# sidfeels/cosmos-predict2.5

Measured on AMD Instinct MI355X. Metric: frames/sec, Predict2.5-2B Image2World 720p×121f, 35 UniPC steps, CP=1/8, higher is better.
Workload: dtype bf16

## Files before the change

cosmos-predict2.5_amd/csrc/attn_wide.hip:

```cpp
#include "attn_common.h"

namespace cp25attn {
namespace {

constexpr int kAheadWq = 2;
constexpr int kRingWq = kAheadWq + 1;
static_assert(kWqThreads == 4 * 64, "one wave per SIMD");

constexpr int wq_stage(int nq) { return 17 * nq; }
constexpr int wq_frag(int nq, int m) { return m < nq ? -1 : (m - nq) / nq; }
constexpr int wq_qb(int nq, int m) { return m < nq ? m : (m - nq) % nq; }
constexpr bool wq_read_gap(int nq, int m) { return m >= nq && (m - nq) % nq == 0; }
constexpr int wq_sm_op(int nq, int m) {
  if (wq_read_gap(nq, m)) return -1;
  int idx = 0;
  for (int x = 0; x < m; ++x) idx += !wq_read_gap(nq, x);
  return idx < 12 * nq ? idx : -1;
}
constexpr int wq_sm_count(int nq) {
  int n = 0;
  for (int m = 0; m < wq_stage(nq); ++m) n += wq_sm_op(nq, m) >= 0;
  return n;
}
static_assert(wq_sm_count(5) == 60 && wq_sm_count(6) == 72, "every softmax instruction has a gap");
constexpr int wq_dma_at(int nq, int M) {
  return M < wq_stage(nq) && wq_read_gap(nq, M) && wq_frag(nq, M) < 10 ? wq_frag(nq, M) : -1;
}
constexpr int wq_m0_at(int nq, int M) { return wq_dma_at(nq, M + 1); }

__device__ __forceinline__ u32x4 tile_rsrc(const char* base, int64_t sl, int rows) {
  const uint64_t p = (uint64_t)base;
  const unsigned n = rows > 0 ? (unsigned)((rows - 1) * sl * 2 + 2 * kD) : 0u;
  return u32x4{(unsigned)p, (unsigned)(p >> 32) & 0xffffu, n, 0x00020000u};
}

#define WQ_MFMA "v_mfma_f32_16x16x32_bf16 "

template <int kNQ, int kMode, int kTail = 0>
__global__ void __launch_bounds__(kWqThreads, 1) attn_fwd_wq(AttnArgs a) {
  static_assert(kMode == 0 || kMode == 1, "kMode: 0 fixed shift, 1 zero shift");
  static_assert(kNQ >= 4 && kNQ <= 6, "query blocks per wave");
  __shared__ __attribute__((aligned(16))) char smem[kLds16];
  constexpr bool kInit = kMode != 1;
  constexpr int KB1 = kKBuf16, VB0 = 2 * kKBuf16;
  constexpr int kR = kRingWq;
  constexpr int kRowsW = 16 * kNQ;
  constexpr int kRowsG = 4 * kRowsW;
  constexpr int kNS = wq_stage(kNQ);
  constexpr int kQA = (256 - 36 * kNQ - 4) / 16 < kNQ ? (256 - 36 * kNQ - 4) / 16 : kNQ;

  const int tile = xcd_remap(blockIdx.x, gridDim.x);
  const int qblk = tile % a.nqb;
  const int bhs = tile / a.nqb;
  const int split = bhs % a.nsplit, bh = bhs / a.nsplit;
  const int b = bh / a.H, h = bh % a.H;
  const int key0 = split * a.tps * kKBlk;
  const int Lk = min(a.Lk - key0, a.tps * kKBlk);
  const int ntk = (Lk + kKBlk - 1) / kKBlk;
  const int tid = threadIdx.x;
  const int lane = tid & 63;
  const int wave = __builtin_amdgcn_readfirstlane(tid >> 6);
  const int c16 = lane & 15;
  const int g = lane >> 4;
  const int row_w = qblk * kRowsG + wave * kRowsW;

  const unsigned short* qp = a.q + b * a.q_sb + h * a.q_sh;
  const char* const kbase = (const char*)(a.k + b * a.k_sb + h * a.k_sh + (int64_t)key0 * a.k_sl);
  const char* const vbase = (const char*)(a.v + b * a.v_sb + h * a.v_sh + (int64_t)key0 * a.v_sl);

  int dk[5], dv[5];
#pragma unroll
  for (int j = 0; j < 5; ++j) {
    const int bb = 1024 * (wave + 4 * j) + 16 * lane;
    const int row = bb / kKStride16, cb = bb - row * kKStride16;
    dk[j] = cb < 2 * kD ? row * (int)(a.k_sl * 2) + cb : 0;
    dv[j] = cb < 2 * kD ? row * (int)(a.v_sl * 2) + cb : 0;
  }
  const unsigned lds_wave = (unsigned)(uintptr_t)(lds_char_ptr)smem + 1024u * (unsigned)wave;
  auto k_rsrc = [&](int t) __attribute__((always_inline)) {
    return tile_rsrc(kbase + (int64_t)t * kKBlk * a.k_sl * 2, a.k_sl, min(Lk - t * kKBlk, kKBlk));
  };
  auto v_rsrc = [&](int t) __attribute__((always_inline)) {
    return tile_rsrc(vbase + (int64_t)t * kKBlk * a.v_sl * 2, a.v_sl, min(Lk - t * kKBlk, kKBlk));
  };
  auto set_m0 = [&](unsigned dst, auto OFFC) __attribute__((always_inline)) {
    asm volatile("s_add_u32 m0, %0, %1" ::"s"(dst), "i"(decltype(OFFC)::value) : "memory");
  };
  auto dma_load = [&](const u32x4& rs, int off) __attribute__((always_inline)) {
    asm volatile("buffer_load_dwordx4 %0, %1, 0 offen lds" ::"v"(off), "s"(rs) : "memory");
  };
  auto dma_tile = [&](const u32x4& rs, const int* offs, unsigned dst) __attribute__((always_inline)) {
    static_for<5>([&](auto JC) __attribute__((always_inline)) {
      constexpr int j = decltype(JC)::value;
      if (j < 4 || wave < 2) {
        set_m0(dst, std::integral_constant<int, 4096 * j>{});
        asm volatile("s_nop 0" ::: "memory");
        dma_load(rs, offs[j]);
      }
    });
  };

  dma_tile(k_rsrc(0), dk, lds_wave);
  dma_tile(k_rsrc(1), dk, lds_wave + KB1);
  dma_tile(v_rsrc(0), dv, lds_wave + VB0);

  bf16x8 qa[kNQ][4];
#pragma unroll
  for (int qb = 0; qb < kNQ; ++qb) {
    const int r = row_w + 16 * qb + c16;
    const unsigned short* src = qp + (int64_t)min(r, a.Lq - 1) * a.q_sl + 8 * g;
#pragma unroll
    for (int s = 0; s < 4; ++s) qa[qb][s] = *reinterpret_cast<const bf16x8*>(src + 32 * s);
  }
  if (a.qn_w != nullptr) {
    bf16x8 wv[4];
#pragma unroll
    for (int s = 0; s < 4; ++s) wv[s] = *reinterpret_cast<const bf16x8*>(a.qn_w + 32 * s + 8 * g);
    const bool rope = a.qn_cos != nullptr;
    const f32x2 scale2 = {a.qn_scale, a.qn_scale};
#pragma unroll
    for (int qb = 0; qb < kNQ; ++qb) {
      const int r = row_w + 16 * qb + c16;
      f32x4 rc[2][2], rsn[2][2];
      if (rope) {
        const int64_t t0 = (a.qn_row0 + min(r, a.Lq - 1)) * 64 + 8 * g;
#pragma unroll
        for (int s1 = 0; s1 < 2; ++s1)
#pragma unroll
          for (int hf = 0; hf < 2; ++hf) {
            rc[s1][hf] = *reinterpret_cast<const f32x4*>(a.qn_cos + t0 + 32 * s1 + 4 * hf);
            rsn[s1][hf] = *reinterpret_cast<const f32x4*>(a.qn_sin + t0 + 32 * s1 + 4 * hf);
          }
      }
      f32x2 x[4][4];
#pragma unroll
      for (int s = 0; s < 4; ++s)
#pragma unroll
        for (int q = 0; q < 4; ++q)
          x[s][q] = f32x2{static_cast<float>(qa[qb][s][2 * q]), static_cast<float>(qa[qb][s][2 * q + 1])};
      f32x2 c01[8], c23[8];
#pragma unroll
      for (int e = 0; e < 8; ++e) {
        c01[e] = f32x2{x[0][e >> 1][e & 1], x[1][e >> 1][e & 1]};
        c23[e] = f32x2{x[2][e >> 1][e & 1], x[3][e >> 1][e & 1]};
      }
      const f32x2 p01 = hn2_sumsq8(c01), p23 = hn2_sumsq8(c23);
      const f32x2 aa = p01 + p23;
      float ss = aa.x + aa.y;
      ss += __shfl_xor(ss, 32);
      ss += __shfl_xor(ss, 16);
      const float rstd = hn_rstd(ss, a.qn_eps);
      const f32x2 rstd2 = {rstd, rstd};
#pragma unroll
      for (int s = 0; s < 4; ++s)
#pragma unroll
        for (int q = 0; q < 4; ++q)
          x[s][q] = hn2_norm(x[s][q], rstd2,
                             f32x2{static_cast<float>(wv[s][2 * q]), static_cast<float>(wv[s][2 * q + 1])});
      f32x2 y[4][4];
#pragma unroll
      for (int s = 0; s < 4; ++s)
#pragma unroll
        for (int q = 0; q < 4; ++q) y[s][q] = x[s][q];
      if (rope) {
#pragma unroll
        for (int s = 0; s < 4; ++s)
#pragma unroll
          for (int q = 0; q < 4; ++q) {
            const f32x4 cc = rc[s & 1][q >> 1], sn = rsn[s & 1][q >> 1];
            const int o = 2 * (q & 1);
            y[s][q] = hn2_rope(x[s][q], x[s ^ 2][q], s < 2 ? -1.f : 1.f, f32x2{cc[o], cc[o + 1]},
                               f32x2{sn[o], sn[o + 1]});
          }
      }
#pragma unroll
      for (int s = 0; s < 4; ++s)
#pragma unroll
        for (int q = 0; q < 4; ++q) {
          const bf16x2v hh = __builtin_convertvector(y[s][q] * scale2, bf16x2v);
          qa[qb][s][2 * q] = hh.x;
          qa[qb][s][2 * q + 1] = hh.y;
        }
    }
  }

  float m_run[kNQ];
#pragma unroll
  for (int qb = 0; qb < kNQ; ++qb) m_run[qb] = 0.f;
  if constexpr (kMode == 0) {
#pragma unroll
    for (int qb = 0; qb < kNQ; ++qb) {
      float qq = 0.f;
#pragma unroll
      for (int s = 0; s < 4; ++s)
#pragma unroll
        for (int e = 0; e < 8; ++e) {
          const float x = static_cast<float>(qa[qb][s][e]);
          qq = fmaf(x, x, qq);
        }
      const float b_row = sqrtf(group4_sum(qq)) * a.kbound;
      m_run[qb] = floorf(fminf(b_row + kPDrop, 126.f - b_row));
    }
  }
  f32x4 minit[kNQ];
#pragma unroll
  for (int qb = 0; qb < kNQ; ++qb) {
    minit[qb] = f32x4{-m_run[qb], -m_run[qb], -m_run[qb], -m_run[qb]};
    asm volatile("" : "+v"(minit[qb]));
  }

  f32x4 oacc[8][kNQ], lacc[kNQ];
#pragma unroll
  for (int db = 0; db < 8; ++db)
#pragma unroll
    for (int qb = 0; qb < kNQ; ++qb) {
      oacc[db][qb] = f32x4{0.f, 0.f, 0.f, 0.f};
      asm volatile("s_nop 2" : "+a"(oacc[db][qb]));
    }
#pragma unroll
  for (int qb = 0; qb < kNQ; ++qb) {
    lacc[qb] = f32x4{0.f, 0.f, 0.f, 0.f};
    asm volatile("s_nop 2" : "+a"(lacc[qb]));
  }
  static_for<kNQ>([&](auto QC) __attribute__((always_inline)) {
    constexpr int qb = decltype(QC)::value;
    (void)qa;
#pragma unroll
    for (int s = 0; s < 4; ++s) {
      if constexpr (qb < kQA) asm volatile("s_nop 2" : "+a"(qa[qb][s]));
      else asm volatile("s_nop 2" : "+v"(qa[qb][s]));
    }
  });
  typedef short s16x8v __attribute__((ext_vector_type(8)));
  bf16x8 ones8 = __builtin_bit_cast(bf16x8, s16x8v{0x3f80, 0x3f80, 0x3f80, 0x3f80, 0x3f80, 0x3f80, 0x3f80, 0x3f80});
  asm volatile("s_nop 2" : "+a"(ones8));
  const unsigned k_rd_lds = (unsigned)(uintptr_t)(lds_char_ptr)(smem + c16 * kKStride16 + 16 * g);
  const unsigned v_rd_lds =
      (unsigned)(uintptr_t)(lds_char_ptr)(smem + VB0 + (4 * g + (c16 >> 2)) * kVStride16 + 8 * (c16 & 3));

  f32x4 S[2][2][kNQ];
  bf16x8 P[2][kNQ];
  bf16x8 ring[kR];
  float ex[2];
  unsigned pk[4];
  unsigned k_cur = 0, v_cur = 0;

  auto issue = [&](auto FC, auto SLOTC) __attribute__((always_inline)) {
    constexpr int F = decltype(FC)::value, slot = decltype(SLOTC)::value;
    constexpr int st = F / 16, f = F % 16;
    (void)ring;
    (void)k_cur;
    (void)v_cur;
    if constexpr (f >= 8) {
      constexpr int j = f - 8;
      constexpr int off = (2 * st + (j & 1)) * 16 * kKStride16 + 64 * (j >> 1);
      asm volatile("ds_read_b128 %0, %1 offset:%2" : "=v"(ring[slot]) : "v"(k_cur), "i"(off));
    } else {
      constexpr int off = 32 * st * kVStride16 + 32 * f;
      s16x4 lo, hi;
      asm volatile("ds_read_b64_tr_b16 %0, %1 offset:%2" : "=v"(lo) : "v"(v_cur), "i"(off));
      asm volatile("ds_read_b64_tr_b16 %0, %1 offset:%2" : "=v"(hi) : "v"(v_cur), "i"(off + 16 * kVStride16));
      typedef short s16x8 __attribute__((ext_vector_type(8)));
      const s16x8 r = {lo[0], lo[1], lo[2], lo[3], hi[0], hi[1], hi[2], hi[3]};
      ring[slot] = __builtin_bit_cast(bf16x8, r);
    }
  };

  auto mask_keys = [&](auto SPC, int k0) __attribute__((always_inline)) {
    constexpr int SP = decltype(SPC)::value;
    if (__builtin_expect(k0 + 32 > Lk, 0)) {
      asm volatile("s_nop 15\n\ts_nop 15" ::: "memory");
#pragma unroll
      for (int kbl = 0; kbl < 2; ++kbl)
#pragma unroll
        for (int i = 0; i < 4; ++i)
          if (k0 + 16 * kbl + 4 * g + i >= Lk) {
#pragma unroll
            for (int qb = 0; qb < kNQ; ++qb) S[SP][kbl][qb][i] = -INFINITY;
          }
    }
  };

  auto body = [&](auto FULLC, int t) __attribute__((always_inline)) {
    constexpr bool FULL = decltype(FULLC)::value;
    constexpr int NF = FULL ? 32 : 16;
    constexpr auto frag_of = [](int n) constexpr { return FULL ? n : (n < 8 ? 8 + n : 16 + n); };
    constexpr auto seq_of = [](int F) constexpr { return FULL ? F : (F < 16 ? F - 8 : F - 16); };
    constexpr auto nreads = [](int F) constexpr { return F % 16 < 8 ? 2 : 1; };
    k_cur = k_rd_lds + (((t + 1) & 1) ? (unsigned)KB1 : 0u);
    v_cur = v_rd_lds + ((t & 1) ? (unsigned)kVBuf16 : 0u);
    u32x4 rk = {0u, 0u, 0u, 0u}, rv = {0u, 0u, 0u, 0u};
    unsigned dst_k = 0, dst_v = 0;
    if constexpr (FULL) {
      mask_keys(std::integral_constant<int, 1>{}, 64 * t + 32);
      rk = k_rsrc(t + 2);
      rv = v_rsrc(t + 1);
      dst_k = lds_wave + ((t & 1) ? (unsigned)KB1 : 0u);
      dst_v = lds_wave + (unsigned)VB0 + (((t + 1) & 1) ? (unsigned)kVBuf16 : 0u);
    }
    static_for<kAheadWq>([&](auto IC) __attribute__((always_inline)) {
      constexpr int n = decltype(IC)::value;
      issue(std::integral_constant<int, frag_of(n)>{}, std::integral_constant<int, n % kR>{});
    });
    __builtin_amdgcn_sched_barrier(0);
    static_for<2 * kNS>([&](auto MC) __attribute__((always_inline)) {
      constexpr int M = decltype(MC)::value;
      constexpr int st = M / kNS, m = M % kNS;
      constexpr int f = wq_frag(kNQ, m), qb = wq_qb(kNQ, m);
      constexpr int F = 16 * st + (f < 0 ? 0 : f);
      constexpr bool has_mfma = f >= 8 || FULL;
      constexpr bool has_sm = st == 1 || FULL;
      (void)S;
      (void)ex;
      (void)pk;
      (void)oacc;
      (void)lacc;
      (void)ones8;
      (void)P;
      (void)minit;
      (void)qa;
      (void)ring;
      (void)rk;
      (void)rv;
      (void)dst_k;
      (void)dst_v;
      if constexpr (m == 0 && st == 1) {
        if constexpr (!FULL) asm volatile("s_nop 15" ::: "memory");
        mask_keys(std::integral_constant<int, 0>{}, 64 * (t + 1));
        __builtin_amdgcn_sched_barrier(0);
      }
      if constexpr (has_mfma) {
        if constexpr (f >= 0 && qb == 0) {
          constexpr int n = seq_of(F);
          constexpr int pending = [=]() constexpr {
            int p = 0;
            for (int i = 1; i < kAheadWq; ++i)
              if (n + i < NF) p += nreads(frag_of(n + i));
            return p;
          }();
          asm volatile("s_waitcnt lgkmcnt(%0)" ::"i"(pending), "v"(ring[n % kR]) : "memory");
        }
        if constexpr (f < 0) {
          asm volatile(WQ_MFMA "%0, %1, %2, %0" : "+a"(lacc[qb]) : "a"(ones8), "v"(P[st][qb]));
        } else if constexpr (f < 8) {
          asm volatile(WQ_MFMA "%0, %1, %2, %0" : "+a"(oacc[f][qb]) : "v"(ring[seq_of(F) % kR]), "v"(P[st][qb]));
        } else {
          constexpr int kbl = (f - 8) & 1, s = (f - 8) >> 1;
          constexpr int ri = seq_of(F) % kR;
          if constexpr (qb < kQA) {
            if constexpr (s == 0 && kInit)
              asm volatile(WQ_MFMA "%0, %1, %2, %3"
                           : "=&v"(S[st][kbl][qb]) : "v"(ring[ri]), "a"(qa[qb][s]), "v"(minit[qb]));
            else if constexpr (s == 0)
              asm volatile(WQ_MFMA "%0, %1, %2, 0" : "=&v"(S[st][kbl][qb]) : "v"(ring[ri]), "a"(qa[qb][s]));
            else
              asm volatile(WQ_MFMA "%0, %1, %2, %0" : "+v"(S[st][kbl][qb]) : "v"(ring[ri]), "a"(qa[qb][s]));
          } else {
            if constexpr (s == 0 && kInit)
              asm volatile(WQ_MFMA "%0, %1, %2, %3"
                           : "=&v"(S[st][kbl][qb]) : "v"(ring[ri]), "v"(qa[qb][s]), "v"(minit[qb]));
            else if constexpr (s == 0)
              asm volatile(WQ_MFMA "%0, %1, %2, 0" : "=&v"(S[st][kbl][qb]) : "v"(ring[ri]), "v"(qa[qb][s]));
            else
              asm volatile(WQ_MFMA "%0, %1, %2, %0" : "+v"(S[st][kbl][qb]) : "v"(ring[ri]), "v"(qa[qb][s]));
          }
        }
      }
      __builtin_amdgcn_sched_barrier(0);
      if constexpr (has_mfma && f >= 0 && qb == 0) {
        constexpr int n = seq_of(F) + kAheadWq;
        if constexpr (n < NF) issue(std::integral_constant<int, frag_of(n)>{}, std::integral_constant<int, n % kR>{});
      }
      if constexpr (FULL) {
        constexpr int dm = wq_m0_at(kNQ, M), dl = wq_dma_at(kNQ, M);
        if constexpr (dm >= 0) {
          constexpr int j = dm % 5;
          if (j < 4 || wave < 2) set_m0(dm < 5 ? dst_k : dst_v, std::integral_constant<int, 4096 * j>{});
        }
        if constexpr (dl >= 0) {
          constexpr int j = dl % 5;
          if (j < 4 || wave < 2) dma_load(dl < 5 ? rk : rv, dl < 5 ? dk[j] : dv[j]);
        }
      }
      if constexpr (has_sm) {
        if constexpr (!has_mfma) asm volatile("s_nop 1" ::: "memory");
        constexpr int op = wq_sm_op(kNQ, m);
        if constexpr (op >= 0) {
          constexpr int q = op / 12, r = op % 12, pair = r / 3, w = r % 3;
          if constexpr (w < 2) {
            constexpr int j = 2 * pair + w;
            asm volatile("v_exp_f32 %0, %1" : "=v"(ex[w]) : "v"(S[1 - st][j >> 2][q][j & 3]));
          } else {
            pk[pair] = __builtin_bit_cast(unsigned, __builtin_convertvector(f32x2{ex[0], ex[1]}, bf16x2v));
            asm volatile("" ::"v"(pk[pair]));
            if constexpr (pair == 3) P[1 - st][q] = __builtin_bit_cast(bf16x8, u32x4{pk[0], pk[1], pk[2], pk[3]});
          }
        }
      }
      __builtin_amdgcn_sched_barrier(0);
    });
    if constexpr (FULL) {
      static_for<kNQ>([&](auto QC) __attribute__((always_inline)) {
        constexpr int qb = decltype(QC)::value;
        (void)P;
        asm volatile("" ::"v"(P[0][qb]), "v"(P[1][qb]));
      });
    }
    asm volatile("s_waitcnt vmcnt(0)" ::: "memory");
    __builtin_amdgcn_s_barrier();
    __builtin_amdgcn_sched_barrier(0);
  };

  asm volatile("s_waitcnt vmcnt(0) lgkmcnt(0)" ::: "memory");
  __builtin_amdgcn_s_barrier();
  body(std::false_type{}, -1);
  for (int t = 0; t < ntk; ++t) body(std::true_type{}, t);

  asm volatile("s_nop 15\n\ts_nop 15" ::: "memory");
#pragma unroll
  for (int db = 0; db < 8; ++db)
#pragma unroll
    for (int qb = 0; qb < kNQ; ++qb) asm volatile("s_nop 0" : "+a"(oacc[db][qb]));
#pragma unroll
  for (int qb = 0; qb < kNQ; ++qb) asm volatile("s_nop 0" : "+a"(lacc[qb]));
#pragma unroll
  for (int qb = 0; qb < kNQ; ++qb) {
    const int q_row = row_w + 16 * qb + c16;
    const float l_tot = lacc[qb][0];
    float inv = 1.f / l_tot;
    if (l_tot > 3.0e38f) inv = __uint_as_float(0x7fc00000u);
    if (q_row >= a.Lq) continue;
    if (a.nsplit > 1) {
      const int64_t row = ((int64_t)(split * a.B + b) * a.H + h) * a.Lq + q_row;
      float* op = a.o_part + row * kD + 4 * g;
#pragma unroll
      for (int db = 0; db < 8; ++db) {
        f32x4 w;
#pragma unroll
        for (int e = 0; e < 4; ++e) w[e] = oacc[db][qb][e] * inv;
        *reinterpret_cast<f32x4*>(op + 16 * db) = w;
      }
      if (g == 0) a.lse_part[row] = m_run[qb] + __log2f(l_tot);
    } else {
      unsigned short* op = a.o + b * a.o_sb + h * a.o_sh + (int64_t)q_row * a.o_sl + 4 * g;
#pragma unroll
      for (int db = 0; db < 8; ++db) {
        u16x4 w;
#pragma unroll
        for (int e = 0; e < 4; ++e) w[e] = f2bf(oacc[db][qb][e] * inv);
        *reinterpret_cast<u16x4*>(op + 16 * db) = w;
      }
    }
  }
}

#undef WQ_MFMA

}

AttnKernel wq_kernel(int rows, int mode, bool tail) {
  if (mode != 0) return nullptr;
  if (rows == 320) return tail ? attn_fwd_wq<5, 0, 1> : attn_fwd_wq<5, 0>;
  if (rows == 384) return tail ? attn_fwd_wq<6, 0, 1> : attn_fwd_wq<6, 0>;
  return nullptr;
}

}
```

Before: 0.7987.

## Process two key tiles per barrier iteration in wide-query attention kernel

Restructures the attention main loop so each iteration consumes two K/V tiles instead of one, doubling the LDS staging buffers and halving the number of s_waitcnt/s_barrier synchronisations per key range. The DMA schedule is regenerated for 18 loads per iteration, with the fifth (partial) image piece split across wave pairs. Buffer resource descriptors are computed at the iteration head by default. The goal is less barrier and pipeline-drain overhead, at the cost of more LDS, longer unrolled code and a new tile-count rounding for odd tile counts.

```diff
diff --git a/cosmos-predict2.5_amd/csrc/attn_wide.hip b/cosmos-predict2.5_amd/csrc/attn_wide.hip
--- a/cosmos-predict2.5_amd/csrc/attn_wide.hip
+++ b/cosmos-predict2.5_amd/csrc/attn_wide.hip
@@ -23,10 +23,36 @@
   return n;
 }
 static_assert(wq_sm_count(5) == 60 && wq_sm_count(6) == 72, "every softmax instruction has a gap");
-constexpr int wq_dma_at(int nq, int M) {
-  return M < wq_stage(nq) && wq_read_gap(nq, M) && wq_frag(nq, M) < 10 ? wq_frag(nq, M) : -1;
-}
-constexpr int wq_m0_at(int nq, int M) { return wq_dma_at(nq, M + 1); }
+#ifdef CP25_WQ_PARENT_LOOP
+#define CP25_WQ_ITER_TILES 1
+#undef CP25_WQ_NO_PAD_FETCH
+#undef CP25_WQ_GAP_RSRC
+#endif
+#ifndef CP25_WQ_ITER_TILES
+#define CP25_WQ_ITER_TILES 2
+#endif
+constexpr int wq_iter_tiles(int) { return CP25_WQ_ITER_TILES; }
+#ifdef CP25_WQ_NO_PAD_FETCH
+constexpr bool kWqPadFetch = false;
+#else
+constexpr bool kWqPadFetch = true;
+#endif
+#ifdef CP25_WQ_GAP_RSRC
+constexpr bool kWqHeadRsrc = false;
+#else
+constexpr bool kWqHeadRsrc = true;
+#endif
+constexpr int kWqImg = kKBuf16;
+static_assert(kKBuf16 == kVBuf16, "K and V images of one size");
+constexpr int wq_dma_n(int it) { return it == 1 ? 10 : 18; }
+constexpr int wq_dma_at(int nq, int it, int M) {
+  const int st = M / wq_stage(nq), m = M % wq_stage(nq);
+  if (st >= 2 * it || !wq_read_gap(nq, m)) return -1;
+  const int F = 16 * st + wq_frag(nq, m);
+  return F < wq_dma_n(it) ? F : -1;
+}
+constexpr int wq_m0_at(int nq, int it, int M) { return wq_dma_at(nq, it, M + 1); }
+constexpr int kWqNoFetch = 0x7ffffff0;
 
 __device__ __forceinline__ u32x4 tile_rsrc(const char* base, int64_t sl, int rows) {
   const uint64_t p = (uint64_t)base;
@@ -40,9 +66,15 @@
 __global__ void __launch_bounds__(kWqThreads, 1) attn_fwd_wq(AttnArgs a) {
   static_assert(kMode == 0 || kMode == 1, "kMode: 0 fixed shift, 1 zero shift");
   static_assert(kNQ >= 4 && kNQ <= 6, "query blocks per wave");
-  __shared__ __attribute__((aligned(16))) char smem[kLds16];
+  constexpr int kIT = wq_iter_tiles(kNQ);
+  static_assert(kIT == 1 || kIT == 2, "tiles per iteration");
+  constexpr int kBuf = kIT * kWqImg;
+  constexpr int VB0 = 2 * kBuf;
+  static_assert(4 * kBuf <= 163840, "the CU's LDS");
+  __shared__ __attribute__((aligned(16))) char smem[4 * kBuf];
   constexpr bool kInit = kMode != 1;
-  constexpr int KB1 = kKBuf16, VB0 = 2 * kKBuf16;
+  constexpr int kPar = kIT == 1 ? 1 : 0;
+  constexpr int kND = wq_dma_n(kIT);
   constexpr int kR = kRingWq;
   constexpr int kRowsW = 16 * kNQ;
   constexpr int kRowsG = 4 * kRowsW;
@@ -68,15 +100,19 @@
   const char* const kbase = (const char*)(a.k + b * a.k_sb + h * a.k_sh + (int64_t)key0 * a.k_sl);
   const char* const vbase = (const char*)(a.v + b * a.v_sb + h * a.v_sh + (int64_t)key0 * a.v_sl);
 
+  const int wave5 = kIT == 1 ? wave : (wave & 1);
+  const int img5 = kIT == 1 ? 0 : (wave >> 1);
   int dk[5], dv[5];
 #pragma unroll
   for (int j = 0; j < 5; ++j) {
-    const int bb = 1024 * (wave + 4 * j) + 16 * lane;
+    const int bb = 1024 * ((j < 4 ? wave : wave5) + 4 * j) + 16 * lane;
     const int row = bb / kKStride16, cb = bb - row * kKStride16;
-    dk[j] = cb < 2 * kD ? row * (int)(a.k_sl * 2) + cb : 0;
-    dv[j] = cb < 2 * kD ? row * (int)(a.v_sl * 2) + cb : 0;
+    dk[j] = cb < 2 * kD ? row * (int)(a.k_sl * 2) + cb : (kWqPadFetch ? 0 : kWqNoFetch);
+    dv[j] = cb < 2 * kD ? row * (int)(a.v_sl * 2) + cb : (kWqPadFetch ? 0 : kWqNoFetch);
   }
   const unsigned lds_wave = (unsigned)(uintptr_t)(lds_char_ptr)smem + 1024u * (unsigned)wave;
+  const unsigned lds_wave5 =
+      (unsigned)(uintptr_t)(lds_char_ptr)smem + 1024u * (unsigned)wave5 + (unsigned)kWqImg * (unsigned)img5;
   auto k_rsrc = [&](int t) __attribute__((always_inline)) {
     return tile_rsrc(kbase + (int64_t)t * kKBlk * a.k_sl * 2, a.k_sl, min(Lk - t * kKBlk, kKBlk));
   };
@@ -84,25 +120,43 @@
     return tile_rsrc(vbase + (int64_t)t * kKBlk * a.v_sl * 2, a.v_sl, min(Lk - t * kKBlk, kKBlk));
   };
   auto set_m0 = [&](unsigned dst, auto OFFC) __attribute__((always_inline)) {
-    asm volatile("s_add_u32 m0, %0, %1" ::"s"(dst), "i"(decltype(OFFC)::value) : "memory");
+    asm volatile("s_add_u32 m0, %0, %1" ::"s"(dst), "i"(decltype(OFFC)::value) : "memory", "scc");
   };
   auto dma_load = [&](const u32x4& rs, int off) __attribute__((always_inline)) {
     asm volatile("buffer_load_dwordx4 %0, %1, 0 offen lds" ::"v"(off), "s"(rs) : "memory");
   };
-  auto dma_tile = [&](const u32x4& rs, const int* offs, unsigned dst) __attribute__((always_inline)) {
-    static_for<5>([&](auto JC) __attribute__((always_inline)) {
-      constexpr int j = decltype(JC)::value;
-      if (j < 4 || wave < 2) {
-        set_m0(dst, std::integral_constant<int, 4096 * j>{});
-        asm volatile("s_nop 0" ::: "memory");
-        dma_load(rs, offs[j]);
-      }
+  auto dma_piece = [&](const u32x4& rs, int off, unsigned dst, auto OFFC) __attribute__((always_inline)) {
+    set_m0(dst, OFFC);
+    asm volatile("s_nop 4" ::: "memory");
+    dma_load(rs, off);
+  };
+  auto dma_img = [&](const u32x4& rs, const int* offs, unsigned at) __attribute__((always_inline)) {
+    static_for<4>([&](auto JC) __attribute__((always_inline)) {
+      dma_piece(rs, offs[decltype(JC)::value], lds_wave + at, std::integral_constant<int, 4096 * decltype(JC)::value>{});
     });
   };
-
-  dma_tile(k_rsrc(0), dk, lds_wave);
-  dma_tile(k_rsrc(1), dk, lds_wave + KB1);
-  dma_tile(v_rsrc(0), dv, lds_wave + VB0);
+  auto dma_buf = [&](auto rsrc, const int* offs, int t0, unsigned at) __attribute__((always_inline)) {
+    if constexpr (kIT == 1) {
+      const u32x4 rs = rsrc(t0);
+      dma_img(rs, offs, at);
+      if (wave < 2) dma_piece(rs, offs[4], lds_wave + at, std::integral_constant<int, 16384>{});
+    } else {
+      const u32x4 rs0 = rsrc(t0), rs1 = rsrc(t0 + 1);
+      dma_img(rs0, offs, at);
+      dma_img(rs1, offs, at + (unsigned)kWqImg);
+      if (wave < 2) dma_piece(rs0, offs[4], lds_wave5 + at, std::integral_constant<int, 16384>{});
+      else dma_piece(rs1, offs[4], lds_wave5 + at, std::integral_constant<int, 16384>{});
+    }
+  };
+
+  constexpr unsigned kK0At = (unsigned)(((kPar + 1) & 1) * kBuf + (kIT - 1) * kWqImg);
+  {
+    const u32x4 rs = k_rsrc(0);
+    dma_img(rs, dk, kK0At);
+    if (wave < 2) dma_piece(rs, dk[4], lds_wave + kK0At, std::integral_constant<int, 16384>{});
+  }
+  dma_buf(k_rsrc, dk, 1, (unsigned)((kPar & 1) * kBuf));
+  dma_buf(v_rsrc, dv, 0, (unsigned)VB0);
 
   bf16x8 qa[kNQ][4];
 #pragma unroll
@@ -248,15 +302,17 @@
   auto issue = [&](auto FC, auto SLOTC) __attribute__((always_inline)) {
     constexpr int F = decltype(FC)::value, slot = decltype(SLOTC)::value;
     constexpr int st = F / 16, f = F % 16;
+    constexpr int img = (st >> 1) * kWqImg, hs = st & 1;
+    static_assert(img + kWqImg <= 65536, "ds_read offset field");
     (void)ring;
     (void)k_cur;
     (void)v_cur;
     if constexpr (f >= 8) {
       constexpr int j = f - 8;
-      constexpr int off = (2 * st + (j & 1)) * 16 * kKStride16 + 64 * (j >> 1);
+      constexpr int off = img + (2 * hs + (j & 1)) * 16 * kKStride16 + 64 * (j >> 1);
       asm volatile("ds_read_b128 %0, %1 offset:%2" : "=v"(ring[slot]) : "v"(k_cur), "i"(off));
     } else {
-      constexpr int off = 32 * st * kVStride16 + 32 * f;
+      constexpr int off = img + 32 * hs * kVStride16 + 32 * f;
       s16x4 lo, hi;
       asm volatile("ds_read_b64_tr_b16 %0, %1 offset:%2" : "=v"(lo) : "v"(v_cur), "i"(off));
       asm volatile("ds_read_b64_tr_b16 %0, %1 offset:%2" : "=v"(hi) : "v"(v_cur), "i"(off + 16 * kVStride16));
@@ -281,35 +337,112 @@
     }
   };
 
+  u32x4 rk[kIT], rv[kIT], rk5 = {0u, 0u, 0u, 0u}, rv5 = {0u, 0u, 0u, 0u};
+  const int64_t kstep = (int64_t)kKBlk * a.k_sl * 2, vstep = (int64_t)kKBlk * a.v_sl * 2;
+  const char* kp = kbase + (kIT + 1) * kstep;
+  const char* vp = vbase + kIT * vstep;
+  int rows_k = Lk - (kIT + 1) * kKBlk, rows_v = Lk - kIT * kKBlk;
+  auto dma_next = [&](auto CC) __attribute__((always_inline)) {
+    constexpr int c = decltype(CC)::value;
+    if constexpr (c == 0) {
+#pragma unroll
+      for (int i = 0; i < kIT; ++i) rk[i] = tile_rsrc(kp + i * kstep, a.k_sl, min(rows_k - i * kKBlk, kKBlk));
+      kp += kIT * kstep;
+      rows_k -= kIT * kKBlk;
+    } else if constexpr (c == 1) {
+#pragma unroll
+      for (int i = 0; i < kIT; ++i) rv[i] = tile_rsrc(vp + i * vstep, a.v_sl, min(rows_v - i * kKBlk, kKBlk));
+      vp += kIT * vstep;
+      rows_v -= kIT * kKBlk;
+    } else if constexpr (kIT == 2) {
+#pragma unroll
+      for (int e = 0; e < 4; ++e) {
+        rk5[e] = img5 ? rk[kIT - 1][e] : rk[0][e];
+        rv5[e] = img5 ? rv[kIT - 1][e] : rv[0][e];
+      }
+    }
+  };
+  if constexpr (!kWqHeadRsrc) static_for<3>(dma_next);
+  constexpr int kNextAt = (2 * kIT - 1) * wq_stage(kNQ) + wq_stage(kNQ) - 3;
+  static_assert(!wq_read_gap(kNQ, wq_stage(kNQ) - 3) && !wq_read_gap(kNQ, wq_stage(kNQ) - 2) &&
+                    !wq_read_gap(kNQ, wq_stage(kNQ) - 1) && wq_sm_op(kNQ, wq_stage(kNQ) - 3) < 0,
+                "a stage's last three gaps carry no read and no softmax instruction");
+
   auto body = [&](auto FULLC, int t) __attribute__((always_inline)) {
     constexpr bool FULL = decltype(FULLC)::value;
-    constexpr int NF = FULL ? 32 : 16;
+    constexpr int NST = FULL ? 2 * kIT : 2;
+    constexpr int NF = FULL ? 16 * NST : 16;
     constexpr auto frag_of = [](int n) constexpr { return FULL ? n : (n < 8 ? 8 + n : 16 + n); };
     constexpr auto seq_of = [](int F) constexpr { return FULL ? F : (F < 16 ? F - 8 : F - 16); };
     constexpr auto nreads = [](int F) constexpr { return F % 16 < 8 ? 2 : 1; };
-    k_cur = k_rd_lds + (((t + 1) & 1) ? (unsigned)KB1 : 0u);
-    v_cur = v_rd_lds + ((t & 1) ? (unsigned)kVBuf16 : 0u);
-    u32x4 rk = {0u, 0u, 0u, 0u}, rv = {0u, 0u, 0u, 0u};
-    unsigned dst_k = 0, dst_v = 0;
+    const int key_sm = FULL ? 64 * kIT * t + 32 : -32;
+    unsigned dst_k = 0, dst_v = 0, dst_k5 = 0, dst_v5 = 0;
     if constexpr (FULL) {
-      mask_keys(std::integral_constant<int, 1>{}, 64 * t + 32);
-      rk = k_rsrc(t + 2);
-      rv = v_rsrc(t + 1);
-      dst_k = lds_wave + ((t & 1) ? (unsigned)KB1 : 0u);
-      dst_v = lds_wave + (unsigned)VB0 + (((t + 1) & 1) ? (unsigned)kVBuf16 : 0u);
-    }
+      k_cur = k_rd_lds + (((t + kPar) & 1) ? (unsigned)kBuf : 0u);
+      v_cur = v_rd_lds + ((t & 1) ? (unsigned)kBuf : 0u);
+      mask_keys(std::integral_constant<int, 1>{}, key_sm);
+      if constexpr (kWqHeadRsrc) {
+#pragma unroll
+        for (int i = 0; i < kIT; ++i) {
+          rk[i] = k_rsrc(kIT * (t + 1) + 1 + i);
+          rv[i] = v_rsrc(kIT * (t + 1) + i);
+        }
+        if constexpr (kIT == 2) dma_next(std::integral_constant<int, 2>{});
+      }
+      const unsigned at_k = ((t + 1 + kPar) & 1) ? (unsigned)kBuf : 0u;
+      const unsigned at_v = (unsigned)VB0 + (((t + 1) & 1) ? (unsigned)kBuf : 0u);
+      dst_k = lds_wave + at_k;
+      dst_v = lds_wave + at_v;
+      if constexpr (kIT == 2) {
+        dst_k5 = lds_wave5 + at_k;
+        dst_v5 = lds_wave5 + at_v;
+      }
+    } else {
+      k_cur = k_rd_lds + kK0At;
+      v_cur = v_rd_lds;
+    }
+    auto dma_m0 = [&](auto DC) __attribute__((always_inline)) {
+      constexpr int d = decltype(DC)::value, i = d % (kND / 2);
+      constexpr bool isk = d < kND / 2;
+      (void)dst_k;
+      (void)dst_v;
+      (void)dst_k5;
+      (void)dst_v5;
+      if constexpr (kIT == 1) {
+        if (i < 4 || wave < 2) set_m0(isk ? dst_k : dst_v, std::integral_constant<int, 4096 * i>{});
+      } else if constexpr (i < 8) {
+        set_m0(isk ? dst_k : dst_v, std::integral_constant<int, (i / 4) * kWqImg + 4096 * (i % 4)>{});
+      } else {
+        set_m0(isk ? dst_k5 : dst_v5, std::integral_constant<int, 16384>{});
+      }
+    };
+    auto dma_ld = [&](auto DC) __attribute__((always_inline)) {
+      constexpr int d = decltype(DC)::value, i = d % (kND / 2);
+      constexpr bool isk = d < kND / 2;
+      (void)rk;
+      (void)rv;
+      (void)rk5;
+      (void)rv5;
+      if constexpr (kIT == 1) {
+        if (i < 4 || wave < 2) dma_load(isk ? rk[0] : rv[0], isk ? dk[i] : dv[i]);
+      } else if constexpr (i < 8) {
+        dma_load(isk ? rk[i / 4] : rv[i / 4], isk ? dk[i % 4] : dv[i % 4]);
+      } else {
+        dma_load(isk ? rk5 : rv5, isk ? dk[4] : dv[4]);
+      }
+    };
     static_for<kAheadWq>([&](auto IC) __attribute__((always_inline)) {
       constexpr int n = decltype(IC)::value;
       issue(std::integral_constant<int, frag_of(n)>{}, std::integral_constant<int, n % kR>{});
     });
     __builtin_amdgcn_sched_barrier(0);
-    static_for<2 * kNS>([&](auto MC) __attribute__((always_inline)) {
+    static_for<NST * kNS>([&](auto MC) __attribute__((always_inline)) {
       constexpr int M = decltype(MC)::value;
-      constexpr int st = M / kNS, m = M % kNS;
+      constexpr int st = M / kNS, m = M % kNS, hs = st & 1;
       constexpr int f = wq_frag(kNQ, m), qb = wq_qb(kNQ, m);
       constexpr int F = 16 * st + (f < 0 ? 0 : f);
       constexpr bool has_mfma = f >= 8 || FULL;
-      constexpr bool has_sm = st == 1 || FULL;
+      constexpr bool has_sm = st >= 1 || FULL;
       (void)S;
       (void)ex;
       (void)pk;
@@ -320,13 +453,9 @@
       (void)minit;
       (void)qa;
       (void)ring;
-      (void)rk;
-      (void)rv;
-      (void)dst_k;
-      (void)dst_v;
-      if constexpr (m == 0 && st == 1) {
+      if constexpr (m == 0 && st >= 1) {
         if constexpr (!FULL) asm volatile("s_nop 15" ::: "memory");
-        mask_keys(std::integral_constant<int, 0>{}, 64 * (t + 1));
+        mask_keys(std::integral_constant<int, 1 - hs>{}, key_sm + 32 * st);
         __builtin_amdgcn_sched_barrier(0);
       }
       if constexpr (has_mfma) {
@@ -341,28 +470,28 @@
           asm volatile("s_waitcnt lgkmcnt(%0)" ::"i"(pending), "v"(ring[n % kR]) : "memory");
         }
         if constexpr (f < 0) {
-          asm volatile(WQ_MFMA "%0, %1, %2, %0" : "+a"(lacc[qb]) : "a"(ones8), "v"(P[st][qb]));
+          asm volatile(WQ_MFMA "%0, %1, %2, %0" : "+a"(lacc[qb]) : "a"(ones8), "v"(P[hs][qb]));
         } else if constexpr (f < 8) {
-          asm volatile(WQ_MFMA "%0, %1, %2, %0" : "+a"(oacc[f][qb]) : "v"(ring[seq_of(F) % kR]), "v"(P[st][qb]));
+          asm volatile(WQ_MFMA "%0, %1, %2, %0" : "+a"(oacc[f][qb]) : "v"(ring[seq_of(F) % kR]), "v"(P[hs][qb]));
         } else {
           constexpr int kbl = (f - 8) & 1, s = (f - 8) >> 1;
           constexpr int ri = seq_of(F) % kR;
           if constexpr (qb < kQA) {
             if constexpr (s == 0 && kInit)
               asm volatile(WQ_MFMA "%0, %1, %2, %3"
-                           : "=&v"(S[st][kbl][qb]) : "v"(ring[ri]), "a"(qa[qb][s]), "v"(minit[qb]));
+                           : "=&v"(S[hs][kbl][qb]) : "v"(ring[ri]), "a"(qa[qb][s]), "v"(minit[qb]));
             else if constexpr (s == 0)
-              asm volatile(WQ_MFMA "%0, %1, %2, 0" : "=&v"(S[st][kbl][qb]) : "v"(ring[ri]), "a"(qa[qb][s]));
+              asm volatile(WQ_MFMA "%0, %1, %2, 0" : "=&v"(S[hs][kbl][qb]) : "v"(ring[ri]), "a"(qa[qb][s]));
             else
-              asm volatile(WQ_MFMA "%0, %1, %2, %0" : "+v"(S[st][kbl][qb]) : "v"(ring[ri]), "a"(qa[qb][s]));
+              asm volatile(WQ_MFMA "%0, %1, %2, %0" : "+v"(S[hs][kbl][qb]) : "v"(ring[ri]), "a"(qa[qb][s]));
           } else {
             if constexpr (s == 0 && kInit)
               asm volatile(WQ_MFMA "%0, %1, %2, %3"
-                           : "=&v"(S[st][kbl][qb]) : "v"(ring[ri]), "v"(qa[qb][s]), "v"(minit[qb]));
+                           : "=&v"(S[hs][kbl][qb]) : "v"(ring[ri]), "v"(qa[qb][s]), "v"(minit[qb]));
             else if constexpr (s == 0)
-              asm volatile(WQ_MFMA "%0, %1, %2, 0" : "=&v"(S[st][kbl][qb]) : "v"(ring[ri]), "v"(qa[qb][s]));
+              asm volatile(WQ_MFMA "%0, %1, %2, 0" : "=&v"(S[hs][kbl][qb]) : "v"(ring[ri]), "v"(qa[qb][s]));
             else
-              asm volatile(WQ_MFMA "%0, %1, %2, %0" : "+v"(S[st][kbl][qb]) : "v"(ring[ri]), "v"(qa[qb][s]));
+              asm volatile(WQ_MFMA "%0, %1, %2, %0" : "+v"(S[hs][kbl][qb]) : "v"(ring[ri]), "v"(qa[qb][s]));
           }
         }
       }
@@ -372,15 +501,11 @@
         if constexpr (n < NF) issue(std::integral_constant<int, frag_of(n)>{}, std::integral_constant<int, n % kR>{});
       }
       if constexpr (FULL) {
-        constexpr int dm = wq_m0_at(kNQ, M), dl = wq_dma_at(kNQ, M);
-        if constexpr (dm >= 0) {
-          constexpr int j = dm % 5;
-          if (j < 4 || wave < 2) set_m0(dm < 5 ? dst_k : dst_v, std::integral_constant<int, 4096 * j>{});
-        }
-        if constexpr (dl >= 0) {
-          constexpr int j = dl % 5;
-          if (j < 4 || wave < 2) dma_load(dl < 5 ? rk : rv, dl < 5 ? dk[j] : dv[j]);
-        }
+        constexpr int dm = wq_m0_at(kNQ, kIT, M), dl = wq_dma_at(kNQ, kIT, M);
+        if constexpr (dm >= 0) dma_m0(std::integral_constant<int, dm>{});
+        if constexpr (dl >= 0) dma_ld(std::integral_constant<int, dl>{});
+        if constexpr (!kWqHeadRsrc && M >= kNextAt && M < kNextAt + 3)
+          dma_next(std::integral_constant<int, M - kNextAt>{});
       }
       if constexpr (has_sm) {
         if constexpr (!has_mfma) asm volatile("s_nop 1" ::: "memory");
@@ -389,11 +514,11 @@
           constexpr int q = op / 12, r = op % 12, pair = r / 3, w = r % 3;
           if constexpr (w < 2) {
             constexpr int j = 2 * pair + w;
-            asm volatile("v_exp_f32 %0, %1" : "=v"(ex[w]) : "v"(S[1 - st][j >> 2][q][j & 3]));
+            asm volatile("v_exp_f32 %0, %1" : "=v"(ex[w]) : "v"(S[1 - hs][j >> 2][q][j & 3]));
           } else {
             pk[pair] = __builtin_bit_cast(unsigned, __builtin_convertvector(f32x2{ex[0], ex[1]}, bf16x2v));
             asm volatile("" ::"v"(pk[pair]));
-            if constexpr (pair == 3) P[1 - st][q] = __builtin_bit_cast(bf16x8, u32x4{pk[0], pk[1], pk[2], pk[3]});
+            if constexpr (pair == 3) P[1 - hs][q] = __builtin_bit_cast(bf16x8, u32x4{pk[0], pk[1], pk[2], pk[3]});
           }
         }
       }
@@ -414,7 +539,8 @@
   asm volatile("s_waitcnt vmcnt(0) lgkmcnt(0)" ::: "memory");
   __builtin_amdgcn_s_barrier();
   body(std::false_type{}, -1);
-  for (int t = 0; t < ntk; ++t) body(std::true_type{}, t);
+  const int nit = (ntk + kIT - 1) / kIT;
+  for (int t = 0; t < nit; ++t) body(std::true_type{}, t);
 
   asm volatile("s_nop 15\n\ts_nop 15" ::: "memory");
 #pragma unroll
```

After: 0.8155, median of 6. +2.1%, better.
